# CC834/Heterogeneous-OpenCL-Image-Processing-Engine

Hardware: AMD Instinct MI355X
Metric: images_per_sec (higher is better)
Workload: dtype u8

## Files before the change

heterogeneous-opencl-image-processing-engine_amd/csrc/blur_launch.h:

```cpp
#pragma once
#include <hip/hip_runtime.h>
#include <stdint.h>

#include "filter.h"

namespace mi_blur {

struct LaunchDesc {
    const Filter *filter;
    const uint8_t *in;
    uint8_t *out;
    int width, band_rows, channels;
    int n_images;
    int y0, y1;
    long long in_stride, out_stride;
    int concurrent;
    int max_blocks;
    int variant;
    const uint8_t *halo_top, *halo_bottom;
    hipStream_t stream;
    hipEvent_t start, stop;
};

int launch(const LaunchDesc &d);
// ... 23 lines not shown
constexpr unsigned ZC_PARAM_WORDS = 32;
constexpr unsigned ZC_TRACE_BATCHES = 512;
constexpr unsigned long long ZC_HARD_TICKS = 1000000000ull;
struct ZcBatch {
    unsigned params[ZC_PARAM_WORDS];
    unsigned tile_first;
    unsigned n_tiles;
    unsigned pad[6];
};
struct ZcHostCtl {
    unsigned tail;
    unsigned quit;
    unsigned servers_done;
    unsigned error;
    unsigned pad0[12];
    unsigned done[ZC_RING];
    unsigned long long t_begin[ZC_RING], t_end[ZC_RING];
    ZcBatch batch[ZC_RING];
};
struct ZcDevCtl {
    unsigned next[2];
    unsigned gnext[2];
    unsigned start_seq;
    unsigned avail;
    unsigned stop_seq, stop_at, stop_tile;
    unsigned ticket;
    unsigned pad[6];
    unsigned tiles_done[ZC_RING];
    ZcBatch batch[ZC_RING];
};
struct ZcGeometry { unsigned threads; size_t lds; int rpg; int channels, radius, ragged; };
int zc_fill_batch(const LaunchDesc &d, ZcGeometry *geo, ZcBatch *b, unsigned *n_tiles);
int zc_launch_server(const ZcGeometry &geo, ZcHostCtl *ctl, ZcDevCtl *dev, unsigned seq, unsigned n_workers, unsigned budget,
                     unsigned idle_ticks, hipStream_t stream, unsigned long long *trace = nullptr, int fixed_share = 0);

const char *last_kernel();

bool tiled_eligible(const void *in, const void *out, int width, int channels);

struct Tunables {
    int stage_dma; int rpg; int xcd_remap; int debug_copy; int row_shuffle; int prefer_stream; int stream_bh; int zero_copy; int ragged;
    int fused_release;
    int experiment;
    int xcd_run;
    int zero_copy_streams;
    int zero_copy_blocks;
    int stream_updown;
    int prefer_direct;
    int direct_bh;
    int debug_xcd_times;
    int fused_window;
    int fused_tail;
    int fused_adds_per_word;
    int fused_tail_blocks;
    int zero_copy_server;
    int zero_copy_server_min_kb;
    int staged_server;
    int zero_copy_workers;
    int zero_copy_idle_us;
    int zero_copy_budget;
    int zero_copy_tickets;
    int resident_place_trials;
    int zero_copy_spin;
    int zero_copy_trace;
    int zero_copy_debug_base;
    int zero_copy_events;
};
enum class KnobKind { FLAG, RANGE, ONE_OF };
struct Knob { const char *key; int Tunables::*field; KnobKind kind; int lo, hi, def; const char *env; };
constexpr int knob_bits(int a, int b, int c, int d) { return 1 << a | 1 << b | 1 << c | 1 << d; }
static constexpr Knob KNOBS[] = {
    {"stage_dma", &Tunables::stage_dma, KnobKind::FLAG, 0, 1, 1, "MI_BLUR_STAGE"},
    {"rows_per_thread", &Tunables::rpg, KnobKind::ONE_OF, knob_bits(0, 4, 8, 16), 0, 0, "MI_BLUR_RPG"},
    {"xcd_remap", &Tunables::xcd_remap, KnobKind::FLAG, 0, 1, 1, "MI_BLUR_XCD"},
    {"debug_copy", &Tunables::debug_copy, KnobKind::FLAG, 0, 1, 0, nullptr},
    {"row_shuffle", &Tunables::row_shuffle, KnobKind::FLAG, 0, 1, 0, nullptr},
    {"prefer_stream", &Tunables::prefer_stream, KnobKind::FLAG, 0, 1, 0, nullptr},
    {"zero_copy", &Tunables::zero_copy, KnobKind::FLAG, 0, 1, 1, nullptr},
    {"ragged_tiled", &Tunables::ragged, KnobKind::FLAG, 0, 1, 1, nullptr},
    {"stream_band_rows", &Tunables::stream_bh, KnobKind::RANGE, 0, 4096, 0, nullptr},
    {"fused_release", &Tunables::fused_release, KnobKind::FLAG, 0, 1, 0, nullptr},
    {"experiment", &Tunables::experiment, KnobKind::FLAG, 0, 1, 0, nullptr},
    {"stream_updown", &Tunables::stream_updown, KnobKind::FLAG, 0, 1, 1, nullptr},
    {"zero_copy_streams", &Tunables::zero_copy_streams, KnobKind::RANGE, 1, 8, 4, nullptr},
    {"zero_copy_blocks", &Tunables::zero_copy_blocks, KnobKind::RANGE, 0, 1 << 20, 24, nullptr},
    {"prefer_direct", &Tunables::prefer_direct, KnobKind::RANGE, 0, 2, 1, "MI_BLUR_DIRECT"},
    {"direct_bh", &Tunables::direct_bh, KnobKind::ONE_OF, knob_bits(4, 8, 12, 16), 0, 8, nullptr},
    {"fused_adds_per_word", &Tunables::fused_adds_per_word, KnobKind::RANGE, 4, 4096, 32, nullptr},
    {"fused_tail_blocks", &Tunables::fused_tail_blocks, KnobKind::RANGE, 10, 800, 25, nullptr},
    {"fused_tail", &Tunables::fused_tail, KnobKind::RANGE, 0, 500, 30, "MI_BLUR_FUSED_TAIL"},
    {"fused_window", &Tunables::fused_window, KnobKind::RANGE, 1, 4096, 8, nullptr},
    {"debug_xcd_times", &Tunables::debug_xcd_times, KnobKind::FLAG, 0, 1, 0, nullptr},
    {"zero_copy_events", &Tunables::zero_copy_events, KnobKind::FLAG, 0, 1, 1, nullptr},
    {"zero_copy_server", &Tunables::zero_copy_server, KnobKind::FLAG, 0, 1, 1, nullptr},
    {"staged_server", &Tunables::staged_server, KnobKind::FLAG, 0, 1, 1, "MI_BLUR_STAGED_SERVER"},
    {"zero_copy_server_min_kb", &Tunables::zero_copy_server_min_kb, KnobKind::RANGE, 0, 1 << 20, 1280, nullptr},
    {"zero_copy_trace", &Tunables::zero_copy_trace, KnobKind::FLAG, 0, 1, 0, nullptr},
    {"zero_copy_tickets", &Tunables::zero_copy_tickets, KnobKind::FLAG, 0, 1, 1, nullptr},
    {"zero_copy_spin", &Tunables::zero_copy_spin, KnobKind::FLAG, 0, 1, 0, nullptr},
    {"zero_copy_debug_base", &Tunables::zero_copy_debug_base, KnobKind::RANGE, 0, 1 << 20, 0, nullptr},
    {"resident_place_trials", &Tunables::resident_place_trials, KnobKind::RANGE, 0, 8, 4, "MI_BLUR_PLACE_TRIALS"},
    {"zero_copy_workers", &Tunables::zero_copy_workers, KnobKind::RANGE, 1, 2048, 48, nullptr},
    {"zero_copy_idle_us", &Tunables::zero_copy_idle_us, KnobKind::RANGE, 10, 100000, 300, nullptr},
    {"zero_copy_budget", &Tunables::zero_copy_budget, KnobKind::RANGE, 1, 1 << 20, 256, nullptr},
    {"xcd_run", &Tunables::xcd_run, KnobKind::RANGE, 0, 1 << 20, 0, nullptr},
};
static inline bool knob_set(const Knob &k, Tunables &t, int value)
{
    switch (k.kind) {
    case KnobKind::FLAG: t.*k.field = value != 0; return true;
    case KnobKind::RANGE: if (value < k.lo || value > k.hi) return false; break;
    case KnobKind::ONE_OF: if (value < 0 || value > 30 || !((k.lo >> value) & 1)) return false; break;
    }
    t.*k.field = value;
    return true;
}

Tunables tunables();
unsigned long long *debug_xcd_buffer();
unsigned debug_xcd_slots();
void set_tunables(const Tunables &t);

}
```

heterogeneous-opencl-image-processing-engine_amd/csrc/mi_blur_api.cpp:

```cpp
#include "../../include/mi_blur.h"
#include "blur_launch.h"
#include "cpu_device.h"

#include <hip/hip_runtime.h>
#include <rccl/rccl.h>

#include <dlfcn.h>
#include <sched.h>
#include <time.h>

#include <algorithm>
#include <chrono>
#include <climits>
#include <cmath>
#include <cstdio>
#include <cstdlib>
#include <cstring>
#include <mutex>
#include <new>
#include <deque>
#include <functional>
#include <condition_variable>
#include <thread>
#include <vector>
// ... 296 lines not shown
                j = q.front(); q.pop_front();
            }
            const auto t0 = std::chrono::steady_clock::now();
            j->work();
            const double ms = std::chrono::duration<double, std::milli>(std::chrono::steady_clock::now() - t0).count();
            { std::lock_guard<std::mutex> lk(m); j->ms = ms; j->done = true; }
            cv_done.notify_all();
        }
    }
    void push(CpuJob *j)
    {
        { std::lock_guard<std::mutex> lk(m); q.push_back(j); }
        if (!th.joinable()) th = std::thread([this] { loop(); });
        cv_work.notify_one();
    }
    void wait(CpuJob *j)
    {
        std::unique_lock<std::mutex> lk(m);
        cv_done.wait(lk, [&] { return j->done; });
    }
    ~CpuWorker()
    {
        { std::lock_guard<std::mutex> lk(m); stop = true; }
        cv_work.notify_all();
        if (th.joinable()) th.join();
    }
};

}

struct mi_blur_ctx {
    int device = 0, W = 0, H = 0, C = 0, max_batch = 0, n_threads = 0;
    Filter filter{};
    size_t image_bytes = 0;
    std::vector<Slot> slots;
    int next_slot = 0;
    mi_blur_timing tm{};
    uint8_t *pool_in = nullptr, *pool_out = nullptr;
    int pool_images = 0;
    long long cursor = 0;
    int rr = 0;
    std::vector<TimedLaunch> ev_pool;
    size_t ev_used = 0;
    uint64_t timed_launches = 0, timed_bytes_alg = 0;
    uint64_t zero_copy_launches = 0;
    hipEvent_t zc_ref = nullptr;
    bool zc_ref_valid = false;
    double zc_covered_ms = 0.0;
    unsigned *fused_count = nullptr, *fused_host = nullptr;
    int fused_cap = 0, fused_batches = 0;
    unsigned fused_tpb = 0, fused_wpb = 0, fused_blocks = 0;
    unsigned fused_k = 8;
    int fused_n = 0, fused_batch = 0;
    unsigned fused_passes = 0;
    hipStream_t fused_poll = nullptr;
    hipStream_t fused_watch = nullptr;
    unsigned long long *fused_word = nullptr, *fused_word_dev = nullptr;
    unsigned fused_watch_seq = 0;
    bool fused_watched = false;
    ZcServer *zc = nullptr;
    std::vector<float> place_ms;
    int place_kept = 0;
    std::vector<CpuJob *> cpu_jobs;
    CpuWorker *cpu_worker = nullptr;
    bool submitted = false;
    bool is_cpu() const { return device == MI_BLUR_DEVICE_CPU; }
};

static bool is_pinned(const void *p)
{
    hipPointerAttribute_t a;
    if (hipPointerGetAttributes(&a, p) != hipSuccess) { (void)hipGetLastError(); return false; }
    return a.type == hipMemoryTypeHost;
}

static uint8_t *pinned_device_ptr(const void *p)
{
    hipPointerAttribute_t a;
    if (hipPointerGetAttributes(&a, p) != hipSuccess) { (void)hipGetLastError(); return nullptr; }
    return a.type == hipMemoryTypeHost ? (uint8_t *)a.devicePointer : nullptr;
}

extern "C" void *mi_blur_host_alloc(size_t bytes)
{
    void *p = nullptr;
    if (mi_blur_device_count() > 0) {
        if (hipHostMalloc(&p, bytes, hipHostMallocPortable | hipHostMallocMapped) == hipSuccess) return p;
        (void)hipGetLastError();
        return nullptr;
    }
    return malloc(bytes);
}

extern "C" int mi_blur_host_register(void *p, size_t bytes)
{
    if (!p || bytes == 0) return MI_BLUR_ERR_INVALID;
    if (mi_blur_device_count() <= 0) return MI_BLUR_OK;
    HIP_TRY(hipHostRegister(p, bytes, hipHostRegisterPortable | hipHostRegisterMapped));
    return MI_BLUR_OK;
}

extern "C" int mi_blur_host_unregister(void *p)
{
    if (!p) return MI_BLUR_ERR_INVALID;
    if (mi_blur_device_count() <= 0) return MI_BLUR_OK;
    HIP_TRY(hipHostUnregister(p));
    return MI_BLUR_OK;
// ... 85 lines not shown
    void *p = nullptr;
    if (hipHostMalloc(&p, bytes, hipHostMallocPortable | hipHostMallocMapped) != hipSuccess) { (void)hipGetLastError(); p = nullptr; }
    if (bound > 0 && have_saved) (void)sched_setaffinity(0, sizeof saved, &saved);
    (void)hipSetDevice(prev);
    return p;
}

static void free_slot(Slot &s)
{
    if (s.h_in) (void)hipHostFree(s.h_in);
    if (s.h_out) (void)hipHostFree(s.h_out);
    if (s.d_in) (void)hipFree(s.d_in);
    if (s.d_out) (void)hipFree(s.d_out);
    for (auto &e : s.ev) if (e) (void)hipEventDestroy(e);
    if (s.ks) (void)hipEventDestroy(s.ks);
    if (s.ke) (void)hipEventDestroy(s.ke);
    if (s.stream) (void)hipStreamDestroy(s.stream);
    s = Slot{};
}

extern "C" int mi_blur_create(mi_blur_ctx **out_ctx, int device, int width, int height, int channels, int radius,
                              int max_batch, int n_slots, int n_threads)
{
    if (!out_ctx) return MI_BLUR_ERR_INVALID;
    *out_ctx = nullptr;
    if (width <= 0 || height <= 0 || channels <= 0 || max_batch <= 0 || n_slots <= 0) return MI_BLUR_ERR_INVALID;
    Filter box;
    if (filter_box(radius, &box)) return MI_BLUR_ERR_INVALID;
    if ((long long)width * channels * height > 0x7fffffffLL) return MI_BLUR_ERR_INVALID;
    mi_blur_ctx *c = new (std::nothrow) mi_blur_ctx;
    if (!c) return MI_BLUR_ERR_NOMEM;
    c->device = device; c->W = width; c->H = height; c->C = channels; c->filter = box;
    c->max_batch = max_batch;
    c->n_threads = n_threads > 0 ? n_threads : std::min(hardware_threads(), 16);
    c->image_bytes = (size_t)width * height * channels;
    if (device == MI_BLUR_DEVICE_CPU) { *out_ctx = c; return MI_BLUR_OK; }

    const int ndev = mi_blur_device_count();
    if (ndev <= 0 || device < 0 || device >= ndev) { delete c; return MI_BLUR_ERR_NO_DEVICE; }
    int rc = MI_BLUR_OK;
    auto fail = [&](hipError_t e) { (void)hipGetLastError(); rc = MI_BLUR_ERR_HIP_BASE - (int)e; return true; };
    hipError_t e = hipSetDevice(device);
    if (e != hipSuccess) { fail(e); delete c; return rc; }
    c->slots.resize(n_slots);
    for (auto &s : c->slots) {
        if ((e = hipStreamCreateWithFlags(&s.stream, hipStreamNonBlocking)) != hipSuccess && fail(e)) break;
        for (auto &ev : s.ev) if ((e = hipEventCreate(&ev)) != hipSuccess && fail(e)) break;
        if (rc) break;
        if ((e = hipEventCreate(&s.ks)) != hipSuccess && fail(e)) break;
        if ((e = hipEventCreate(&s.ke)) != hipSuccess && fail(e)) break;
    }
    if (rc) { mi_blur_destroy(c); return rc; }
    *out_ctx = c;
    return MI_BLUR_OK;
}

static int slot_staging(mi_blur_ctx *c, Slot &s, bool in, bool out)
{
    const size_t bytes = c->image_bytes * (size_t)c->max_batch;
    if (in && !s.h_in) HIP_TRY(hipHostMalloc((void **)&s.h_in, bytes, hipHostMallocDefault));
    if (out && !s.h_out) HIP_TRY(hipHostMalloc((void **)&s.h_out, bytes, hipHostMallocDefault));
    return MI_BLUR_OK;
}
static int slot_device(mi_blur_ctx *c, Slot &s)
{
    const size_t bytes = c->image_bytes * (size_t)c->max_batch;
    if (!s.d_in) HIP_TRY(hipMalloc((void **)&s.d_in, bytes));
    if (!s.d_out) HIP_TRY(hipMalloc((void **)&s.d_out, bytes));
    return MI_BLUR_OK;
}

static int finish_slot(mi_blur_ctx *c, Slot &s)
{
    if (!s.busy) return MI_BLUR_OK;
    float ms = 0.f;
    if (s.zero_copy && s.zc_server) {
        ZcServer &z = *c->zc;
        const unsigned slot = s.zc_index % ZC_RING, want = s.zc_index + 1u;
        const auto t0 = std::chrono::steady_clock::now();
        const bool spin_only = tunables().zero_copy_spin != 0;
        for (unsigned spins = 0; __atomic_load_n(&z.ctl->done[slot], __ATOMIC_ACQUIRE) != want; spins++) {
            if (spins < 2048) { __builtin_ia32_pause(); continue; }
            if (__atomic_load_n(&z.ctl->error, __ATOMIC_ACQUIRE)) return MI_BLUR_ERR_STATE;
            if (spin_only) std::this_thread::yield();
            else { struct timespec ts = {0, 20000}; nanosleep(&ts, nullptr); }
            if ((spins & 63u) == 0) {
                const hipError_t q = hipStreamQuery(z.stream);
                if (q != hipSuccess && q != hipErrorNotReady) { (void)hipGetLastError(); return MI_BLUR_ERR_HIP_BASE - (int)q; }
                (void)hipGetLastError();
                if (std::chrono::steady_clock::now() - t0 > std::chrono::seconds(30)) return MI_BLUR_ERR_STATE;
            }
        }
        const unsigned long long b = __atomic_load_n(&z.ctl->t_begin[slot], __ATOMIC_RELAXED), e = __atomic_load_n(&z.ctl->t_end[slot], __ATOMIC_RELAXED);
        if (e >= b) {
            const unsigned long long from = std::max(b, z.covered);
            if (e > from) c->tm.kernel_ms += (double)(e - from) / 1e5;
            z.covered = std::max(z.covered, e);
        }
        if (s.out_staged)
            copy_blocks(s.user_out, s.out_stride, s.h_out, s.out_band, s.out_band, s.out_n, STAGING_COPY_THREADS);
        s.zero_copy = false; s.zc_server = false; s.busy = false;
        return MI_BLUR_OK;
    }
    if (s.zero_copy) {
        if (s.zc_plain) {
            HIP_TRY(hipStreamSynchronize(s.zc_stream));
            s.zero_copy = false; s.busy = false; s.zc_plain = false;
            return MI_BLUR_OK;
        }
        HIP_TRY(hipEventSynchronize(s.ke));
        float a = 0.f, b = 0.f;
        if (c->zc_ref_valid && hipEventElapsedTime(&a, c->zc_ref, s.ks) == hipSuccess && hipEventElapsedTime(&b, c->zc_ref, s.ke) == hipSuccess && b >= a) {
            const double from = std::max((double)a, c->zc_covered_ms);
            if ((double)b > from) c->tm.kernel_ms += (double)b - from;
            c->zc_covered_ms = std::max(c->zc_covered_ms, (double)b);
        } else if (hipEventElapsedTime(&ms, s.ks, s.ke) == hipSuccess) {
            c->tm.kernel_ms += ms;
        }
        (void)hipGetLastError();
        s.zero_copy = false;
        s.busy = false;
        return MI_BLUR_OK;
    }
    HIP_TRY(hipStreamSynchronize(s.stream));
    if (s.out_staged)
        copy_blocks(s.user_out, s.out_stride, s.h_out, s.out_band, s.out_band, s.out_n, STAGING_COPY_THREADS);
    if (hipEventElapsedTime(&ms, s.ev[0], s.ev[1]) == hipSuccess) c->tm.h2d_ms += ms;
    if (hipEventElapsedTime(&ms, s.ks, s.ke) == hipSuccess) c->tm.kernel_ms += ms;
    if (hipEventElapsedTime(&ms, s.ev[2], s.ev[3]) == hipSuccess) c->tm.d2h_ms += ms;
    (void)hipGetLastError();
    s.busy = false;
    return MI_BLUR_OK;
}

static int harvest_resident(mi_blur_ctx *c)
{
    for (size_t i = 0; i < c->ev_used; i++) {
        float ms = 0.f;
        if (hipEventElapsedTime(&ms, c->ev_pool[i].s, c->ev_pool[i].e) == hipSuccess) c->tm.kernel_ms += ms;
    }
    (void)hipGetLastError();
    c->ev_used = 0;
    return MI_BLUR_OK;
}

extern "C" int mi_blur_sync(mi_blur_ctx *c, mi_blur_timing *timing)
{
    if (!c) return MI_BLUR_ERR_INVALID;
    if (c->is_cpu()) {
        for (CpuJob *j : c->cpu_jobs) {
            c->cpu_worker->wait(j);
            c->tm.kernel_ms += j->ms;
            delete j;
        }
        c->cpu_jobs.clear();
    } else {
        HIP_TRY(hipSetDevice(c->device));
        for (auto &s : c->slots) {
            int rc = finish_slot(c, s);
            if (rc) return rc;
        }
        for (auto &s : c->slots) HIP_TRY(hipStreamSynchronize(s.stream));
        if (c->fused_watched && c->fused_watch) HIP_TRY(hipStreamSynchronize(c->fused_watch));
        harvest_resident(c);
        c->zc_ref_valid = false;
    }
    if (timing) *timing = c->tm;
    return MI_BLUR_OK;
}

extern "C" int mi_blur_get_timing(mi_blur_ctx *c, mi_blur_timing *timing)
{
    if (!c || !timing) return MI_BLUR_ERR_INVALID;
    *timing = c->tm;
    return MI_BLUR_OK;
}

extern "C" uint64_t mi_blur_zero_copy_launches(mi_blur_ctx *c) { return c ? c->zero_copy_launches : 0; }

extern "C" void mi_blur_reset_timing(mi_blur_ctx *c)
{
    if (!c) return;
    c->tm = mi_blur_timing{};
    c->timed_launches = 0; c->timed_bytes_alg = 0;
}

extern "C" void mi_blur_timed_coverage(mi_blur_ctx *c, uint64_t *launches, uint64_t *bytes_alg)
{
    if (launches) *launches = c ? c->timed_launches : 0;
    if (bytes_alg) *bytes_alg = c ? c->timed_bytes_alg : 0;
}

extern "C" void mi_blur_destroy(mi_blur_ctx *c)
{
    if (!c) return;
    for (CpuJob *j : c->cpu_jobs) { c->cpu_worker->wait(j); delete j; }
    delete c->cpu_worker;
    if (!c->is_cpu()) {
        (void)hipSetDevice(c->device);
        for (auto &s : c->slots) { if (s.stream) (void)hipStreamSynchronize(s.stream); }
        if (c->zc) {
            ZcServer &z = *c->zc;
            if (z.ctl) __atomic_store_n(&z.ctl->quit, 1u, __ATOMIC_RELEASE);
            if (getenv("MI_BLUR_DEBUG_SERVER"))
                fprintf(stderr, "[mi_blur] destroy: server state head %u launched %u servers_done %u tail %u; stream query %d\n", z.head, z.launched,
                        z.ctl ? z.ctl->servers_done : 0u, z.ctl ? z.ctl->tail : 0u, z.stream ? (int)hipStreamQuery(z.stream) : -1);
            if (z.stream) { (void)hipStreamSynchronize(z.stream); (void)hipStreamDestroy(z.stream); }
            if (getenv("MI_BLUR_DEBUG_SERVER")) fprintf(stderr, "[mi_blur] destroy: servers gone\n");
            if (z.dev) (void)hipFree(z.dev);
            if (z.trace) (void)hipFree(z.trace);
            if (z.ctl) (void)hipHostFree(z.ctl);
            delete c->zc;
            c->zc = nullptr;
        }
        for (auto &s : c->slots) free_slot(s);
        for (auto &t : c->ev_pool) { (void)hipEventDestroy(t.s); (void)hipEventDestroy(t.e); }
        if (c->zc_ref) (void)hipEventDestroy(c->zc_ref);
        if (c->fused_count) (void)hipFree(c->fused_count);
        if (c->fused_host) (void)hipHostFree(c->fused_host);
        if (c->fused_poll) { (void)hipStreamSynchronize(c->fused_poll); (void)hipStreamDestroy(c->fused_poll); }
        if (c->fused_watch) { (void)hipStreamSynchronize(c->fused_watch); (void)hipStreamDestroy(c->fused_watch); }
        if (c->fused_word) (void)hipHostFree(c->fused_word);
        if (c->pool_in) (void)hipFree(c->pool_in);
        if (c->pool_out) (void)hipFree(c->pool_out);
        (void)hipGetLastError();
    }
    delete c;
}

static int zc_server_submit(mi_blur_ctx *c, Slot &s, const LaunchDesc &d, const Tunables &tun)
{
    if (c->filter.kind != FilterKind::BOX) return MI_BLUR_ERR_UNSUPPORTED;
    if (c->slots.size() > ZC_RING) return MI_BLUR_ERR_UNSUPPORTED;
    if (!c->zc) {
        ZcServer *z = new (std::nothrow) ZcServer;
        if (!z) return MI_BLUR_ERR_NOMEM;
        hipError_t e = hipHostMalloc((void **)&z->ctl, sizeof(ZcHostCtl), hipHostMallocDefault);
        if (e == hipSuccess) { memset(z->ctl, 0, sizeof(ZcHostCtl)); e = hipHostGetDevicePointer((void **)&z->ctl_dev, z->ctl, 0); }
        if (e == hipSuccess) e = hipStreamCreateWithFlags(&z->stream, hipStreamNonBlocking);
        if (e == hipSuccess) e = hipMalloc((void **)&z->dev, sizeof(ZcDevCtl));
        if (e == hipSuccess) e = hipMemsetAsync(z->dev, 0, sizeof(ZcDevCtl), z->stream);
        if (e == hipSuccess && tun.zero_copy_trace) {
            const size_t tb = (size_t)ZC_TRACE_BATCHES * (size_t)tun.zero_copy_workers * 5u * sizeof(unsigned long long);
            e = hipMalloc((void **)&z->trace, tb);
            if (e == hipSuccess) e = hipMemsetAsync(z->trace, 0, tb, z->stream);
        }
        if (e == hipSuccess && tun.zero_copy_debug_base > 0) {
            const unsigned B = 0u - (unsigned)tun.zero_copy_debug_base, T = 0u - 7u * (unsigned)tun.zero_copy_debug_base;
            ZcDevCtl init{};
            init.next[0] = B; init.gnext[0] = T; init.avail = B; init.ticket = T;
            e = hipMemcpyAsync(z->dev, &init, offsetof(ZcDevCtl, tiles_done), hipMemcpyHostToDevice, z->stream);
            if (e == hipSuccess) e = hipStreamSynchronize(z->stream);
            z->ctl->tail = B;
// ... 126 lines not shown
    uint8_t *zout = pinned_device_ptr(s.out_staged ? s.h_out : b.out);
    if (!zin || !zout) return MI_BLUR_ERR_UNSUPPORTED;
    LaunchDesc d = ctx_launch(c, zin, zout, b.band_rows, b.n_images, b.y0, b.y1);
    d.in_stride = (long long)src_stride; d.out_stride = (long long)(s.out_staged ? b.band_out : b.out_stride);
    return submit_to_server(c, s, b, d, tun);
}

static int submit_dma(mi_blur_ctx *c, Slot &s, const HostBatch &b, const uint8_t *src, size_t src_stride)
{
    int rc = slot_device(c, s);
    if (rc) return rc;
    HIP_TRY(hipEventRecord(s.ev[0], s.stream));
    if (src_stride == b.band_in)
        HIP_TRY(hipMemcpyAsync(s.d_in, src, b.in_bytes(), hipMemcpyHostToDevice, s.stream));
    else
        HIP_TRY(hipMemcpy2DAsync(s.d_in, b.band_in, src, src_stride, b.band_in, (size_t)b.n_images, hipMemcpyHostToDevice, s.stream));
    HIP_TRY(hipEventRecord(s.ev[1], s.stream));
    LaunchDesc d = ctx_launch(c, s.d_in, s.d_out, b.band_rows, b.n_images, b.y0, b.y1);
    d.stream = s.stream; d.start = s.ks; d.stop = s.ke;
    d.concurrent = (int)c->slots.size();
    rc = launch(d);
    if (rc) return rc;
    HIP_TRY(hipEventRecord(s.ev[2], s.stream));
    if (s.out_staged || b.out_stride == b.band_out)
        HIP_TRY(hipMemcpyAsync(s.out_staged ? s.h_out : b.out, s.d_out, b.out_bytes(), hipMemcpyDeviceToHost, s.stream));
    else
        HIP_TRY(hipMemcpy2DAsync(b.out, b.out_stride, s.d_out, b.band_out, b.band_out, (size_t)b.n_images, hipMemcpyDeviceToHost, s.stream));
    HIP_TRY(hipEventRecord(s.ev[3], s.stream));
    s.busy = true;
    count_submit(c, b.n_images, b.out_bytes(), b.in_bytes(), b.out_bytes(), false);
    return MI_BLUR_OK;
}

static int submit_common(mi_blur_ctx *c, const uint8_t *host_in, uint8_t *host_out, int band_rows, int n_images,
                         int y0, int y1, size_t in_stride, size_t out_stride)
{
    const size_t pitch = (size_t)c->W * c->C;
    const size_t band_in = pitch * band_rows, band_out = pitch * (size_t)(y1 - y0);
    const HostBatch b{host_in, host_out, band_rows, n_images, y0, y1, band_in, band_out,
                      in_stride ? in_stride : band_in, out_stride ? out_stride : band_out};
    c->submitted = true;
    if (c->is_cpu()) {
        const int W = c->W, C = c->C, nt = c->n_threads;
        const int rc = cpu_enqueue(c, [=, f = c->filter]() {
            cpu_blur_batch(b.in, b.out, W, band_rows, C, f, n_images, y0, y1, nt, b.in_stride, b.out_stride);
        });
        if (rc) return rc;
        count_submit(c, n_images, b.out_bytes(), 0, 0, false);
        return MI_BLUR_OK;
    }
    HIP_TRY(hipSetDevice(c->device));
    Slot &s = c->slots[c->next_slot];
    c->next_slot = (c->next_slot + 1) % (int)c->slots.size();
    int rc = finish_slot(c, s);
    if (rc) return rc;
    const Tunables tun = tunables();
    if (tun.zero_copy) {
        const uint8_t *zin = pinned_device_ptr(host_in);
        uint8_t *zout = pinned_device_ptr(host_out);
        const bool dense = b.in_stride == band_in && b.out_stride == band_out;
        if (zin && zout && (dense || (tiled_eligible(zin, zout, c->W, c->C) && b.in_stride % 16 == 0 && b.out_stride % 16 == 0)))
            return submit_in_place(c, s, b, zin, zout, tun);
    }
    const bool in_pinned = is_pinned(host_in);
    s.zero_copy = false;
    s.out_staged = !is_pinned(host_out);
    s.user_out = host_out; s.out_bytes = b.out_bytes(); s.out_band = band_out; s.out_stride = b.out_stride; s.out_n = n_images;
    const uint8_t *src = host_in;
    size_t src_stride = b.in_stride;
    rc = slot_staging(c, s, !in_pinned, s.out_staged);
    if (rc) return rc;
    if (!in_pinned) {
        copy_blocks(s.h_in, band_in, host_in, b.in_stride, band_in, n_images, STAGING_COPY_THREADS);
        src = s.h_in; src_stride = band_in;
    }
    if (tun.zero_copy && tun.zero_copy_server && tun.staged_server) {
        rc = submit_staged_server(c, s, b, src, src_stride, tun);
        if (rc != MI_BLUR_ERR_UNSUPPORTED) return rc;
    }
    return submit_dma(c, s, b, src, src_stride);
}

extern "C" int mi_blur_submit(mi_blur_ctx *c, const uint8_t *host_in, uint8_t *host_out, int n_images)
{
    if (!c || !host_in || !host_out || host_in == host_out) return MI_BLUR_ERR_INVALID;
    if (n_images < 0 || n_images > c->max_batch) return MI_BLUR_ERR_INVALID;
    if (n_images == 0) return MI_BLUR_OK;
    return submit_common(c, host_in, host_out, c->H, n_images, 0, c->H, 0, 0);
}

extern "C" int mi_blur_submit_band(mi_blur_ctx *c, const uint8_t *host_in, uint8_t *host_out, int band_rows,
                                   int halo_top, int halo_bottom)
{
    if (!c || !host_in || !host_out || host_in == host_out) return MI_BLUR_ERR_INVALID;
    if (band_rows <= 0 || band_rows > c->H || halo_top < 0 || halo_bottom < 0) return MI_BLUR_ERR_INVALID;
    if (halo_top + halo_bottom >= band_rows) return MI_BLUR_ERR_INVALID;
    return submit_common(c, host_in, host_out, band_rows, 1, halo_top, band_rows - halo_bottom, 0, 0);
}

extern "C" int mi_blur_submit_bands(mi_blur_ctx *c, const uint8_t *host_in, uint8_t *host_out, int n_images,
                                    size_t host_image_stride, int band_rows, int halo_top, int halo_bottom)
{
    if (!c || !host_in || !host_out || host_in == host_out) return MI_BLUR_ERR_INVALID;
    if (n_images < 0 || n_images > c->max_batch) return MI_BLUR_ERR_INVALID;
    if (band_rows <= 0 || band_rows > c->H || halo_top < 0 || halo_bottom < 0) return MI_BLUR_ERR_INVALID;
    if (halo_top + halo_bottom >= band_rows) return MI_BLUR_ERR_INVALID;
    if (host_image_stride < (size_t)c->W * c->C * band_rows) return MI_BLUR_ERR_INVALID;
// ... 145 lines not shown
    c->place_ms.clear();
    int keep_in = 0, keep_out = 0;
    if (n_ok > 1) {
        hipStream_t st = c->slots[0].stream;
        hipEvent_t e0 = nullptr, e1 = nullptr;
        std::vector<float> best((size_t)n_ok * n_ok, 1e30f);
        if (hipEventCreate(&e0) == hipSuccess && hipEventCreate(&e1) == hipSuccess) {
            auto pass = [&](int i, int j) {
                LaunchDesc d = ctx_launch(c, in[i], out[j], c->H, pool_images, 0, c->H);
                d.stream = st;
                return launch(d);
            };
            int rc = MI_BLUR_OK;
            const auto t0 = std::chrono::steady_clock::now();
            while (rc == MI_BLUR_OK && std::chrono::steady_clock::now() - t0 < std::chrono::milliseconds(50)) {
                for (int r = 0; r < 4 && rc == MI_BLUR_OK; r++) rc = pass(0, 0);
                if (hipStreamSynchronize(st) != hipSuccess) rc = MI_BLUR_ERR_STATE;
            }
            for (int round = 0; round < 2 && rc == MI_BLUR_OK; round++)
                for (int i = 0; i < n_ok && rc == MI_BLUR_OK; i++)
                    for (int j = 0; j < n_ok && rc == MI_BLUR_OK; j++) {
                        rc = pass(i, j);
                        (void)hipEventRecord(e0, st);
                        for (int r = 0; r < 2 && rc == MI_BLUR_OK; r++) rc = pass(i, j);
                        (void)hipEventRecord(e1, st);
                        float ms = 0.f;
                        if (hipEventSynchronize(e1) == hipSuccess && hipEventElapsedTime(&ms, e0, e1) == hipSuccess && ms > 0.f)
                            best[(size_t)i * n_ok + j] = std::min(best[(size_t)i * n_ok + j], ms / 2.0f);
                    }
            (void)hipGetLastError();
            for (int i = 0; i < n_ok; i++)
                for (int j = 0; j < n_ok; j++) {
                    c->place_ms.push_back(best[(size_t)i * n_ok + j]);
                    if (best[(size_t)i * n_ok + j] < best[(size_t)keep_in * n_ok + keep_out]) { keep_in = i; keep_out = j; }
                }
        }
        if (e0) (void)hipEventDestroy(e0);
        if (e1) (void)hipEventDestroy(e1);
    }
    c->pool_in = in[keep_in]; c->pool_out = out[keep_out];
    c->place_kept = keep_in * n_ok + keep_out;
    for (int i = 0; i < trials; i++) {
        if (i != keep_in && in[i]) (void)hipFree(in[i]);
        if (i != keep_out && out[i]) (void)hipFree(out[i]);
    }
    return MI_BLUR_OK;
}

extern "C" int mi_blur_resident_alloc(mi_blur_ctx *c, int pool_images)
{
    if (!c || pool_images <= 0) return MI_BLUR_ERR_INVALID;
    if (c->is_cpu()) return MI_BLUR_ERR_STATE;
    HIP_TRY(hipSetDevice(c->device));
    if (c->pool_in) { (void)hipFree(c->pool_in); c->pool_in = nullptr; }
    if (c->pool_out) { (void)hipFree(c->pool_out); c->pool_out = nullptr; }
    c->pool_images = 0; c->cursor = 0;
    const size_t bytes = c->image_bytes * (size_t)pool_images;
    const int trials = tunables().resident_place_trials;
    if (trials > 1 && bytes >= ((size_t)128 << 20) && bytes <= ((size_t)8 << 30)) {
        int rc = place_pool(c, bytes, pool_images, std::min(trials, 8));
        if (rc) return rc;
    } else {
        c->place_ms.clear(); c->place_kept = 0;
        HIP_TRY(hipMalloc((void **)&c->pool_in, bytes));
        HIP_TRY(hipMalloc((void **)&c->pool_out, bytes));
    }
    c->pool_images = pool_images;
    return MI_BLUR_OK;
}

extern "C" int mi_blur_resident_placement(mi_blur_ctx *c, float *ms, int max_n, int *kept)
{
    if (!c) return MI_BLUR_ERR_INVALID;
    const int n = (int)std::min<size_t>(c->place_ms.size(), (size_t)std::max(max_n, 0));
    for (int i = 0; i < n && ms; i++) ms[i] = c->place_ms[i];
    if (kept) *kept = c->place_kept;
    return n;
}

extern "C" int mi_blur_resident_upload(mi_blur_ctx *c, int pool_index, const uint8_t *host_in, int n_images)
{
    if (!c || !host_in || !c->pool_in) return MI_BLUR_ERR_STATE;
    if (pool_index < 0 || n_images < 0 || pool_index + n_images > c->pool_images) return MI_BLUR_ERR_INVALID;
    HIP_TRY(hipSetDevice(c->device));
    HIP_TRY(hipMemcpy(c->pool_in + (size_t)pool_index * c->image_bytes, host_in, c->image_bytes * (size_t)n_images,
                      hipMemcpyHostToDevice));
    return MI_BLUR_OK;
}

extern "C" int mi_blur_resident_download(mi_blur_ctx *c, int pool_index, uint8_t *host_out, int n_images)
{
    if (!c || !host_out || !c->pool_out) return MI_BLUR_ERR_STATE;
    if (pool_index < 0 || n_images < 0 || pool_index + n_images > c->pool_images) return MI_BLUR_ERR_INVALID;
    HIP_TRY(hipSetDevice(c->device));
    HIP_TRY(hipDeviceSynchronize());
    HIP_TRY(hipMemcpy(host_out, c->pool_out + (size_t)pool_index * c->image_bytes, c->image_bytes * (size_t)n_images,
                      hipMemcpyDeviceToHost));
    return MI_BLUR_OK;
}

extern "C" int mi_blur_resident_fill_synthetic(mi_blur_ctx *c, int first_index)
{
    if (!c || !c->pool_in) return MI_BLUR_ERR_STATE;
    const int chunk = std::max(1, (int)std::min<size_t>((size_t)c->pool_images, ((size_t)256 << 20) / c->image_bytes));
    std::vector<uint8_t> host;
    try { host.resize(c->image_bytes * (size_t)chunk); } catch (...) { return MI_BLUR_ERR_NOMEM; }
    for (int i = 0; i < c->pool_images; i += chunk) {
        const int n = std::min(chunk, c->pool_images - i);
        fill_synthetic(host.data(), c->W, c->H, c->C, first_index + i, n, c->n_threads);
        int rc = mi_blur_resident_upload(c, i, host.data(), n);
        if (rc) return rc;
    }
    return MI_BLUR_OK;
}

extern "C" void *mi_blur_resident_in(mi_blur_ctx *c) { return c ? c->pool_in : nullptr; }
extern "C" void *mi_blur_resident_out(mi_blur_ctx *c) { return c ? c->pool_out : nullptr; }

extern "C" int mi_blur_resident_run(mi_blur_ctx *c, int n_images, int batch, int timed_every)
{
    if (!c || n_images < 0 || batch <= 0) return MI_BLUR_ERR_INVALID;
    if (c->filter.kind != FilterKind::BOX) return MI_BLUR_ERR_UNSUPPORTED;
    if (c->is_cpu() || !c->pool_in) return MI_BLUR_ERR_STATE;
    if (batch > c->pool_images) return MI_BLUR_ERR_INVALID;
    HIP_TRY(hipSetDevice(c->device));
    int launch_idx = 0;
    for (int done = 0; done < n_images; done += batch, launch_idx++) {
        const int b = std::min(batch, n_images - done);
        const bool timed = timed_every > 0 && launch_idx % timed_every == 0;
        if (c->cursor + b > c->pool_images) c->cursor = 0;
        Slot &s = c->slots[c->rr];
        c->rr = (c->rr + 1) % (int)c->slots.size();
        LaunchDesc d = ctx_launch(c, c->pool_in + (size_t)c->cursor * c->image_bytes, c->pool_out + (size_t)c->cursor * c->image_bytes,
                                  c->H, b, 0, c->H);
        d.stream = s.stream;
        d.concurrent = (int)c->slots.size();
        if (timed) {
            if (c->ev_used == c->ev_pool.size()) {
                TimedLaunch t{};
                HIP_TRY(hipEventCreate(&t.s));
                HIP_TRY(hipEventCreate(&t.e));
                c->ev_pool.push_back(t);
            }
            d.start = c->ev_pool[c->ev_used].s; d.stop = c->ev_pool[c->ev_used].e;
            c->ev_used++;
        }
        int rc = launch(d);
        if (rc) return rc;
        c->cursor += b;
        c->tm.launches += 1;
        if (timed) { c->timed_launches += 1; c->timed_bytes_alg += 2ull * c->image_bytes * (uint64_t)b; }
    }
    c->tm.images += (uint64_t)n_images;
    c->tm.bytes_alg += 2ull * c->image_bytes * (uint64_t)n_images;
    return MI_BLUR_OK;
}

static size_t fused_words(int cap) { return 8 * (size_t)cap + 16384; }

extern "C" int mi_blur_resident_run_fused(mi_blur_ctx *c, int n_images, int batch, int timed)
{
    if (!c || n_images <= 0 || batch <= 0) return MI_BLUR_ERR_INVALID;
    if (c->filter.kind != FilterKind::BOX) return MI_BLUR_ERR_UNSUPPORTED;
    if (c->is_cpu() || !c->pool_in) return MI_BLUR_ERR_STATE;
    if (n_images > c->pool_images) return MI_BLUR_ERR_INVALID;
    HIP_TRY(hipSetDevice(c->device));
    const int nb = (n_images + batch - 1) / batch;
    if (nb > c->fused_cap) {
        for (auto &s : c->slots) HIP_TRY(hipStreamSynchronize(s.stream));
        if (c->fused_count) { (void)hipFree(c->fused_count); c->fused_count = nullptr; }
        if (c->fused_host) { (void)hipHostFree(c->fused_host); c->fused_host = nullptr; }
        c->fused_cap = 0;
        const int cap = std::max(nb, c->pool_images);
        HIP_TRY(hipMalloc((void **)&c->fused_count, sizeof(unsigned) * (fused_words(cap) + 16)));
        HIP_TRY(hipMemset(c->fused_count + fused_words(cap), 0, sizeof(unsigned) * 16));
        HIP_TRY(hipDeviceSynchronize());
        HIP_TRY(hipHostMalloc((void **)&c->fused_host, sizeof(unsigned) * fused_words(cap), hipHostMallocDefault));
        c->fused_cap = cap;
        c->fused_passes = 0;
    }
    if (!c->fused_poll) {
        HIP_TRY(hipStreamCreateWithFlags(&c->fused_poll, hipStreamNonBlocking));
        HIP_TRY(hipMemcpyAsync(c->fused_host, c->fused_count, sizeof(unsigned) * fused_words(c->fused_cap), hipMemcpyDeviceToHost, c->fused_poll));
        HIP_TRY(hipStreamSynchronize(c->fused_poll));
    }
    if (c->cursor + n_images > c->pool_images) c->cursor = 0;
    Slot &s = c->slots[0];
    LaunchDesc d = ctx_launch(c, c->pool_in + (size_t)c->cursor * c->image_bytes, c->pool_out + (size_t)c->cursor * c->image_bytes,
                              c->H, n_images, 0, c->H);
    d.variant = MI_BLUR_VARIANT_TILED; d.stream = s.stream;
    const Tunables tun = tunables();
    unsigned tpb = 0, wpb = 0, blocks = 0, kcnt = 8;
    FusedDesc f{c->fused_count, batch, &tpb, &wpb, &blocks, &tun, true, c->fused_count + fused_words(c->fused_cap), (long long)fused_words(c->fused_cap), &kcnt};
    int rc = launch_fused(d, f);
    if (rc) return rc;
    if (n_images == c->fused_n && batch == c->fused_batch && tpb == c->fused_tpb && wpb == c->fused_wpb && kcnt == c->fused_k &&
        blocks == c->fused_blocks && c->fused_passes > 0 && c->fused_passes < (1u << 20)) {
        c->fused_passes += 1;
    } else {
        if (c->fused_watched && c->fused_watch) HIP_TRY(hipStreamSynchronize(c->fused_watch));
        HIP_TRY(hipMemsetAsync(c->fused_count, 0, sizeof(unsigned) * (size_t)kcnt * (size_t)nb, s.stream));
        c->fused_n = n_images; c->fused_batch = batch; c->fused_passes = 1;
        c->fused_tpb = tpb; c->fused_wpb = wpb; c->fused_blocks = blocks; c->fused_k = kcnt;
    }
    c->fused_batches = nb;
    c->fused_watched = false;
    if (timed & 2) {
        if (c->fused_passes == 1) HIP_TRY(hipStreamSynchronize(s.stream));
        if (!c->fused_watch) HIP_TRY(hipStreamCreateWithFlags(&c->fused_watch, hipStreamNonBlocking));
        if (!c->fused_word) {
            HIP_TRY(hipHostMalloc((void **)&c->fused_word, sizeof(unsigned long long), hipHostMallocDefault));
            *c->fused_word = 0;
            HIP_TRY(hipHostGetDevicePointer((void **)&c->fused_word_dev, c->fused_word, 0));
        }
        c->fused_watch_seq += 1;
        rc = launch_fused_watch(c->fused_count, (unsigned)nb, tpb, blocks, wpb * c->fused_passes, c->fused_word_dev, c->fused_watch_seq, c->fused_watch, c->fused_k);
        if (rc) return rc;
        c->fused_watched = true;
    }
    if (timed & 1) {
        if (c->ev_used == c->ev_pool.size()) {
            TimedLaunch t{};
            HIP_TRY(hipEventCreate(&t.s));
            HIP_TRY(hipEventCreate(&t.e));
            c->ev_pool.push_back(t);
        }
        d.start = c->ev_pool[c->ev_used].s; d.stop = c->ev_pool[c->ev_used].e;
        c->ev_used++;
    }
    f.geometry_only = false;
    rc = launch_fused(d, f);
    if (rc) { c->fused_passes = 0; c->fused_batches = 0; return rc; }
    c->cursor += n_images;
    c->tm.launches += 1;
    c->tm.images += (uint64_t)n_images;
    c->tm.bytes_alg += 2ull * c->image_bytes * (uint64_t)n_images;
    if (timed & 1) { c->timed_launches += 1; c->timed_bytes_alg += 2ull * c->image_bytes * (uint64_t)n_images; }
    return MI_BLUR_OK;
}

extern "C" int mi_blur_resident_batches_done(mi_blur_ctx *c)
{
    if (!c) return MI_BLUR_ERR_INVALID;
    if (c->is_cpu()) return MI_BLUR_ERR_STATE;
    if (!c->fused_count || !c->fused_batches) return 0;
    if (c->fused_watched) {
        const unsigned long long w = __atomic_load_n(c->fused_word, __ATOMIC_ACQUIRE);
        return (unsigned)(w >> 32) == c->fused_watch_seq ? (int)(unsigned)(w & 0xffffffffu) : 0;
    }
    HIP_TRY(hipSetDevice(c->device));
    const unsigned K = c->fused_k;
    HIP_TRY(hipMemcpyAsync(c->fused_host, c->fused_count, sizeof(unsigned) * (size_t)K * (size_t)c->fused_batches, hipMemcpyDeviceToHost, c->fused_poll));
    HIP_TRY(hipStreamSynchronize(c->fused_poll));
    int n = 0;
    for (; n < c->fused_batches; n++) {
        const unsigned first = (unsigned)n * c->fused_tpb;
        const unsigned blocks = std::min(c->fused_tpb, c->fused_blocks - first);
        unsigned sum = 0;
        for (unsigned k = 0; k < K; k++) sum += c->fused_host[(size_t)K * n + k];
        if (sum != blocks * c->fused_wpb * c->fused_passes) break;
    }
    return n;
}

extern "C" int mi_blur_resident_peek(mi_blur_ctx *c, int pool_index, uint8_t *host_out, int n_images)
{
    if (!c || !host_out || !c->pool_out || !c->fused_poll) return MI_BLUR_ERR_STATE;
    if (pool_index < 0 || n_images < 0 || pool_index + n_images > c->pool_images) return MI_BLUR_ERR_INVALID;
    HIP_TRY(hipSetDevice(c->device));
    HIP_TRY(hipMemcpyAsync(host_out, c->pool_out + (size_t)pool_index * c->image_bytes, c->image_bytes * (size_t)n_images,
                           hipMemcpyDeviceToHost, c->fused_poll));
    HIP_TRY(hipStreamSynchronize(c->fused_poll));
    return MI_BLUR_OK;
}

static int cpu_run_filter(const Filter &f, const uint8_t *in, uint8_t *out, int width, int height, int channels, int n_images,
                          int n_threads)
{
    if (!in || !out || in == out || width <= 0 || height <= 0 || channels <= 0 || n_images < 0)
        return MI_BLUR_ERR_INVALID;
    if (f.kind != FilterKind::BOX && (long long)width * channels * height > INT_MAX) return MI_BLUR_ERR_INVALID;
    cpu_blur_batch(in, out, width, height, channels, f, n_images, 0, height, n_threads);
    return MI_BLUR_OK;
}

extern "C" int mi_blur_cpu_run(const uint8_t *in, uint8_t *out, int width, int height, int channels, int radius,
                               int n_images, int n_threads)
{
    Filter f;
    return filter_box(radius, &f) ? MI_BLUR_ERR_INVALID : cpu_run_filter(f, in, out, width, height, channels, n_images, n_threads);
}

extern "C" int mi_blur_cpu_run_sep(const uint8_t *in, uint8_t *out, int width, int height, int channels, int n_images,
                                   const mi_blur_sep_kernel *k, int n_threads)
{
    Filter f;
    return filter_sep(k, &f) ? MI_BLUR_ERR_INVALID : cpu_run_filter(f, in, out, width, height, channels, n_images, n_threads);
}

extern "C" int mi_blur_cpu_run_median(const uint8_t *in, uint8_t *out, int width, int height, int channels, int radius,
                                      int n_images, int n_threads)
{
    Filter f;
    return filter_median(radius, &f) ? MI_BLUR_ERR_INVALID : cpu_run_filter(f, in, out, width, height, channels, n_images, n_threads);
}

extern "C" int mi_blur_cpu_run_morph(const uint8_t *in, uint8_t *out, int width, int height, int channels, int op, int rx, int ry,
                                     int n_images, int n_threads)
{
    Filter f;
    return filter_morph(op, rx, ry, &f) ? MI_BLUR_ERR_INVALID : cpu_run_filter(f, in, out, width, height, channels, n_images, n_threads);
}

// ... 430 lines not shown
```

Before: 15.00 million.

## Add optional dual-lane fused resident launches and cache fused geometry

Adds a fused_lanes knob (default 1) that alternates fused resident launches between two streams, each with its own completion-counter region, so consecutive passes can overlap. Caches the geometry-only launch_fused result keyed on shape, input pointer and tunables, skipping the repeated geometry query. Pre-reserves timing events in bulk instead of creating them on demand. Adds join/synchronization points across the API to keep the second lane coherent, at the cost of extra sync calls and more state.

```diff
diff --git a/heterogeneous-opencl-image-processing-engine_amd/csrc/blur_launch.h b/heterogeneous-opencl-image-processing-engine_amd/csrc/blur_launch.h
--- a/heterogeneous-opencl-image-processing-engine_amd/csrc/blur_launch.h
+++ b/heterogeneous-opencl-image-processing-engine_amd/csrc/blur_launch.h
@@ -99,6 +99,7 @@
     int fused_window;
     int fused_tail;
     int fused_adds_per_word;
+    int fused_lanes;
     int fused_tail_blocks;
     int zero_copy_server;
     int zero_copy_server_min_kb;
@@ -137,6 +138,7 @@
     {"fused_tail_blocks", &Tunables::fused_tail_blocks, KnobKind::RANGE, 10, 800, 25, nullptr},
     {"fused_tail", &Tunables::fused_tail, KnobKind::RANGE, 0, 500, 30, "MI_BLUR_FUSED_TAIL"},
     {"fused_window", &Tunables::fused_window, KnobKind::RANGE, 1, 4096, 8, nullptr},
+    {"fused_lanes", &Tunables::fused_lanes, KnobKind::RANGE, 1, 2, 1, "MI_BLUR_FUSED_LANES"},
     {"debug_xcd_times", &Tunables::debug_xcd_times, KnobKind::FLAG, 0, 1, 0, nullptr},
     {"zero_copy_events", &Tunables::zero_copy_events, KnobKind::FLAG, 0, 1, 1, nullptr},
     {"zero_copy_server", &Tunables::zero_copy_server, KnobKind::FLAG, 0, 1, 1, nullptr},
diff --git a/heterogeneous-opencl-image-processing-engine_amd/csrc/mi_blur_api.cpp b/heterogeneous-opencl-image-processing-engine_amd/csrc/mi_blur_api.cpp
--- a/heterogeneous-opencl-image-processing-engine_amd/csrc/mi_blur_api.cpp
+++ b/heterogeneous-opencl-image-processing-engine_amd/csrc/mi_blur_api.cpp
@@ -372,7 +372,12 @@
     unsigned fused_tpb = 0, fused_wpb = 0, fused_blocks = 0;
     unsigned fused_k = 8;
     int fused_n = 0, fused_batch = 0;
-    unsigned fused_passes = 0;
+    hipStream_t fused_lane1 = nullptr;
+    bool fused_lane1_owned = false;
+    unsigned fused_passes[2] = {0, 0};
+    bool fused_lane1_pending = false;
+    int fused_lane = 1;
+    struct FusedGeo { bool valid = false; int n = 0, batch = 0, radius = 0; const uint8_t *in = nullptr; Tunables tun{}; unsigned tpb = 0, wpb = 0, blocks = 0, k = 8; } fused_geo;
     hipStream_t fused_poll = nullptr;
     hipStream_t fused_watch = nullptr;
     unsigned long long *fused_word = nullptr, *fused_word_dev = nullptr;
@@ -564,6 +569,25 @@
     }
     if (rc) { mi_blur_destroy(c); return rc; }
     *out_ctx = c;
+    return MI_BLUR_OK;
+}
+
+static int fused_join(mi_blur_ctx *c)
+{
+    if (!c->fused_lane1_pending) return MI_BLUR_OK;
+    HIP_TRY(hipStreamSynchronize(c->fused_lane1));
+    c->fused_lane1_pending = false;
+    return MI_BLUR_OK;
+}
+
+static int ev_reserve(mi_blur_ctx *c, size_t n)
+{
+    while (c->ev_pool.size() < n) {
+        TimedLaunch t{};
+        HIP_TRY(hipEventCreate(&t.s));
+        if (hipEventCreate(&t.e) != hipSuccess) { (void)hipEventDestroy(t.s); (void)hipGetLastError(); return MI_BLUR_ERR_STATE; }
+        c->ev_pool.push_back(t);
+    }
     return MI_BLUR_OK;
 }
 
@@ -652,6 +676,7 @@
         if (hipEventElapsedTime(&ms, c->ev_pool[i].s, c->ev_pool[i].e) == hipSuccess) c->tm.kernel_ms += ms;
     }
     (void)hipGetLastError();
+    if (c->ev_used && c->ev_used == c->ev_pool.size() && c->ev_pool.size() < 65536) (void)ev_reserve(c, 2 * c->ev_pool.size());
     c->ev_used = 0;
     return MI_BLUR_OK;
 }
@@ -673,6 +698,7 @@
             if (rc) return rc;
         }
         for (auto &s : c->slots) HIP_TRY(hipStreamSynchronize(s.stream));
+        { int rc = fused_join(c); if (rc) return rc; }
         if (c->fused_watched && c->fused_watch) HIP_TRY(hipStreamSynchronize(c->fused_watch));
         harvest_resident(c);
         c->zc_ref_valid = false;
@@ -693,6 +719,10 @@
 extern "C" void mi_blur_reset_timing(mi_blur_ctx *c)
 {
     if (!c) return;
+    if (!c->is_cpu() && c->fused_lane1_pending && hipSetDevice(c->device) == hipSuccess) {
+        (void)hipStreamSynchronize(c->slots[0].stream);
+        (void)fused_join(c);
+    }
     c->tm = mi_blur_timing{};
     c->timed_launches = 0; c->timed_bytes_alg = 0;
 }
@@ -711,6 +741,7 @@
     if (!c->is_cpu()) {
         (void)hipSetDevice(c->device);
         for (auto &s : c->slots) { if (s.stream) (void)hipStreamSynchronize(s.stream); }
+        if (c->fused_lane1) { (void)hipStreamSynchronize(c->fused_lane1); if (c->fused_lane1_owned) (void)hipStreamDestroy(c->fused_lane1); c->fused_lane1 = nullptr; }
         if (c->zc) {
             ZcServer &z = *c->zc;
             if (z.ctl) __atomic_store_n(&z.ctl->quit, 1u, __ATOMIC_RELEASE);
@@ -943,7 +974,9 @@
     HIP_TRY(hipSetDevice(c->device));
     Slot &s = c->slots[c->next_slot];
     c->next_slot = (c->next_slot + 1) % (int)c->slots.size();
-    int rc = finish_slot(c, s);
+    int rc = fused_join(c);
+    if (rc) return rc;
+    rc = finish_slot(c, s);
     if (rc) return rc;
     const Tunables tun = tunables();
     if (tun.zero_copy) {
@@ -1195,6 +1228,12 @@
     if (!c || pool_images <= 0) return MI_BLUR_ERR_INVALID;
     if (c->is_cpu()) return MI_BLUR_ERR_STATE;
     HIP_TRY(hipSetDevice(c->device));
+    if (c->fused_lane1_pending) {
+        HIP_TRY(hipStreamSynchronize(c->slots[0].stream));
+        int rc = fused_join(c);
+        if (rc) return rc;
+    }
+    c->fused_geo.valid = false;
     if (c->pool_in) { (void)hipFree(c->pool_in); c->pool_in = nullptr; }
     if (c->pool_out) { (void)hipFree(c->pool_out); c->pool_out = nullptr; }
     c->pool_images = 0; c->cursor = 0;
@@ -1209,7 +1248,7 @@
         HIP_TRY(hipMalloc((void **)&c->pool_out, bytes));
     }
     c->pool_images = pool_images;
-    return MI_BLUR_OK;
+    return ev_reserve(c, 256);
 }
 
 extern "C" int mi_blur_resident_placement(mi_blur_ctx *c, float *ms, int max_n, int *kept)
@@ -1226,6 +1265,11 @@
     if (!c || !host_in || !c->pool_in) return MI_BLUR_ERR_STATE;
     if (pool_index < 0 || n_images < 0 || pool_index + n_images > c->pool_images) return MI_BLUR_ERR_INVALID;
     HIP_TRY(hipSetDevice(c->device));
+    if (c->fused_lane1_pending) {
+        HIP_TRY(hipStreamSynchronize(c->slots[0].stream));
+        int rc = fused_join(c);
+        if (rc) return rc;
+    }
     HIP_TRY(hipMemcpy(c->pool_in + (size_t)pool_index * c->image_bytes, host_in, c->image_bytes * (size_t)n_images,
                       hipMemcpyHostToDevice));
     return MI_BLUR_OK;
@@ -1237,6 +1281,7 @@
     if (pool_index < 0 || n_images < 0 || pool_index + n_images > c->pool_images) return MI_BLUR_ERR_INVALID;
     HIP_TRY(hipSetDevice(c->device));
     HIP_TRY(hipDeviceSynchronize());
+    c->fused_lane1_pending = false;
     HIP_TRY(hipMemcpy(host_out, c->pool_out + (size_t)pool_index * c->image_bytes, c->image_bytes * (size_t)n_images,
                       hipMemcpyDeviceToHost));
     return MI_BLUR_OK;
@@ -1267,6 +1312,7 @@
     if (c->is_cpu() || !c->pool_in) return MI_BLUR_ERR_STATE;
     if (batch > c->pool_images) return MI_BLUR_ERR_INVALID;
     HIP_TRY(hipSetDevice(c->device));
+    { int rc = fused_join(c); if (rc) return rc; }
     int launch_idx = 0;
     for (int done = 0; done < n_images; done += batch, launch_idx++) {
         const int b = std::min(batch, n_images - done);
@@ -1279,12 +1325,7 @@
         d.stream = s.stream;
         d.concurrent = (int)c->slots.size();
         if (timed) {
-            if (c->ev_used == c->ev_pool.size()) {
-                TimedLaunch t{};
-                HIP_TRY(hipEventCreate(&t.s));
-                HIP_TRY(hipEventCreate(&t.e));
-                c->ev_pool.push_back(t);
-            }
+            if (c->ev_used == c->ev_pool.size()) { int rc = ev_reserve(c, c->ev_used + 1); if (rc) return rc; }
             d.start = c->ev_pool[c->ev_used].s; d.stop = c->ev_pool[c->ev_used].e;
             c->ev_used++;
         }
@@ -1300,6 +1341,8 @@
 }
 
 static size_t fused_words(int cap) { return 8 * (size_t)cap + 16384; }
+static size_t fused_lane_words(int cap) { return fused_words(cap) + 16; }
+static unsigned *fused_lane_count(const mi_blur_ctx *c, int lane) { return c->fused_count + (size_t)lane * fused_lane_words(c->fused_cap); }
 
 extern "C" int mi_blur_resident_run_fused(mi_blur_ctx *c, int n_images, int batch, int timed)
 {
@@ -1311,16 +1354,20 @@
     const int nb = (n_images + batch - 1) / batch;
     if (nb > c->fused_cap) {
         for (auto &s : c->slots) HIP_TRY(hipStreamSynchronize(s.stream));
+        { int rc = fused_join(c); if (rc) return rc; }
+        if (c->fused_watched && c->fused_watch) HIP_TRY(hipStreamSynchronize(c->fused_watch));
         if (c->fused_count) { (void)hipFree(c->fused_count); c->fused_count = nullptr; }
         if (c->fused_host) { (void)hipHostFree(c->fused_host); c->fused_host = nullptr; }
         c->fused_cap = 0;
         const int cap = std::max(nb, c->pool_images);
-        HIP_TRY(hipMalloc((void **)&c->fused_count, sizeof(unsigned) * (fused_words(cap) + 16)));
+        HIP_TRY(hipMalloc((void **)&c->fused_count, sizeof(unsigned) * 2 * fused_lane_words(cap)));
         HIP_TRY(hipMemset(c->fused_count + fused_words(cap), 0, sizeof(unsigned) * 16));
+        HIP_TRY(hipMemset(c->fused_count + fused_lane_words(cap) + fused_words(cap), 0, sizeof(unsigned) * 16));
         HIP_TRY(hipDeviceSynchronize());
         HIP_TRY(hipHostMalloc((void **)&c->fused_host, sizeof(unsigned) * fused_words(cap), hipHostMallocDefault));
         c->fused_cap = cap;
-        c->fused_passes = 0;
+        c->fused_passes[0] = c->fused_passes[1] = 0;
+        c->fused_batches = 0; c->fused_watched = false;
     }
     if (!c->fused_poll) {
         HIP_TRY(hipStreamCreateWithFlags(&c->fused_poll, hipStreamNonBlocking));
@@ -1328,28 +1375,59 @@
         HIP_TRY(hipStreamSynchronize(c->fused_poll));
     }
     if (c->cursor + n_images > c->pool_images) c->cursor = 0;
-    Slot &s = c->slots[0];
-    LaunchDesc d = ctx_launch(c, c->pool_in + (size_t)c->cursor * c->image_bytes, c->pool_out + (size_t)c->cursor * c->image_bytes,
-                              c->H, n_images, 0, c->H);
-    d.variant = MI_BLUR_VARIANT_TILED; d.stream = s.stream;
+    const uint8_t *in = c->pool_in + (size_t)c->cursor * c->image_bytes;
+    LaunchDesc d = ctx_launch(c, in, c->pool_out + (size_t)c->cursor * c->image_bytes, c->H, n_images, 0, c->H);
+    d.variant = MI_BLUR_VARIANT_TILED;
     const Tunables tun = tunables();
     unsigned tpb = 0, wpb = 0, blocks = 0, kcnt = 8;
-    FusedDesc f{c->fused_count, batch, &tpb, &wpb, &blocks, &tun, true, c->fused_count + fused_words(c->fused_cap), (long long)fused_words(c->fused_cap), &kcnt};
-    int rc = launch_fused(d, f);
-    if (rc) return rc;
-    if (n_images == c->fused_n && batch == c->fused_batch && tpb == c->fused_tpb && wpb == c->fused_wpb && kcnt == c->fused_k &&
-        blocks == c->fused_blocks && c->fused_passes > 0 && c->fused_passes < (1u << 20)) {
-        c->fused_passes += 1;
+    FusedDesc f{nullptr, batch, &tpb, &wpb, &blocks, &tun, true, nullptr, (long long)fused_words(c->fused_cap), &kcnt};
+    auto &g = c->fused_geo;
+    int rc = MI_BLUR_OK;
+    if (g.valid && g.n == n_images && g.batch == batch && g.radius == c->filter.radius && g.in == in && !memcmp(&g.tun, &tun, sizeof tun)) {
+        tpb = g.tpb; wpb = g.wpb; blocks = g.blocks; kcnt = g.k;
+    } else {
+        f.count = c->fused_count; f.tail_ctr = c->fused_count + fused_words(c->fused_cap);
+        rc = launch_fused(d, f);
+        if (rc) return rc;
+        g.valid = true; g.n = n_images; g.batch = batch; g.radius = c->filter.radius; g.in = in; g.tun = tun;
+        g.tpb = tpb; g.wpb = wpb; g.blocks = blocks; g.k = kcnt;
+    }
+    if (!(n_images == c->fused_n && batch == c->fused_batch && tpb == c->fused_tpb && wpb == c->fused_wpb && kcnt == c->fused_k &&
+          blocks == c->fused_blocks)) {
+        if (c->fused_lane1_pending) {
+            HIP_TRY(hipStreamSynchronize(c->slots[0].stream));
+            rc = fused_join(c);
+            if (rc) return rc;
+        }
+        if (c->fused_watched && c->fused_watch) HIP_TRY(hipStreamSynchronize(c->fused_watch));
+        c->fused_passes[0] = c->fused_passes[1] = 0;
+        c->fused_n = n_images; c->fused_batch = batch;
+        c->fused_tpb = tpb; c->fused_wpb = wpb; c->fused_blocks = blocks; c->fused_k = kcnt;
+    }
+    const int lane = tun.fused_lanes >= 2 ? (c->fused_lane ^ 1) : 0;
+    if (lane == 0 && tun.fused_lanes < 2) { rc = fused_join(c); if (rc) return rc; }
+    if (lane && !c->fused_lane1) {
+        if (c->slots.size() >= 2) c->fused_lane1 = c->slots[1].stream;
+        else { HIP_TRY(hipStreamCreateWithFlags(&c->fused_lane1, hipStreamNonBlocking)); c->fused_lane1_owned = true; }
+    }
+    const hipStream_t stream = lane ? c->fused_lane1 : c->slots[0].stream;
+    unsigned *count = fused_lane_count(c, lane);
+    d.stream = stream;
+    f.count = count; f.tail_ctr = count + fused_words(c->fused_cap);
+    unsigned &passes = c->fused_passes[lane];
+    if (passes > 0 && passes < (1u << 20)) {
+        passes += 1;
     } else {
         if (c->fused_watched && c->fused_watch) HIP_TRY(hipStreamSynchronize(c->fused_watch));
-        HIP_TRY(hipMemsetAsync(c->fused_count, 0, sizeof(unsigned) * (size_t)kcnt * (size_t)nb, s.stream));
-        c->fused_n = n_images; c->fused_batch = batch; c->fused_passes = 1;
-        c->fused_tpb = tpb; c->fused_wpb = wpb; c->fused_blocks = blocks; c->fused_k = kcnt;
+        HIP_TRY(hipMemsetAsync(count, 0, sizeof(unsigned) * (size_t)kcnt * (size_t)nb, stream));
+        passes = 1;
     }
     c->fused_batches = nb;
+    c->fused_lane = lane;
     c->fused_watched = false;
-    if (timed & 2) {
-        if (c->fused_passes == 1) HIP_TRY(hipStreamSynchronize(s.stream));
+    if (lane) c->fused_lane1_pending = true;
+    auto watch = [&]() -> int {
+        if (passes == 1) HIP_TRY(hipStreamSynchronize(stream));
         if (!c->fused_watch) HIP_TRY(hipStreamCreateWithFlags(&c->fused_watch, hipStreamNonBlocking));
         if (!c->fused_word) {
             HIP_TRY(hipHostMalloc((void **)&c->fused_word, sizeof(unsigned long long), hipHostMallocDefault));
@@ -1357,23 +1435,22 @@
             HIP_TRY(hipHostGetDevicePointer((void **)&c->fused_word_dev, c->fused_word, 0));
         }
         c->fused_watch_seq += 1;
-        rc = launch_fused_watch(c->fused_count, (unsigned)nb, tpb, blocks, wpb * c->fused_passes, c->fused_word_dev, c->fused_watch_seq, c->fused_watch, c->fused_k);
-        if (rc) return rc;
+        const int wrc = launch_fused_watch(count, (unsigned)nb, tpb, blocks, wpb * passes, c->fused_word_dev, c->fused_watch_seq, c->fused_watch, c->fused_k);
+        if (wrc) return wrc;
         c->fused_watched = true;
-    }
+        return MI_BLUR_OK;
+    };
+    const bool watch_first = tun.fused_lanes < 2;
+    if ((timed & 2) && watch_first) { rc = watch(); if (rc) return rc; }
     if (timed & 1) {
-        if (c->ev_used == c->ev_pool.size()) {
-            TimedLaunch t{};
-            HIP_TRY(hipEventCreate(&t.s));
-            HIP_TRY(hipEventCreate(&t.e));
-            c->ev_pool.push_back(t);
-        }
+        if (c->ev_used == c->ev_pool.size()) { rc = ev_reserve(c, c->ev_used + 1); if (rc) return rc; }
         d.start = c->ev_pool[c->ev_used].s; d.stop = c->ev_pool[c->ev_used].e;
         c->ev_used++;
     }
     f.geometry_only = false;
     rc = launch_fused(d, f);
-    if (rc) { c->fused_passes = 0; c->fused_batches = 0; return rc; }
+    if (rc) { passes = 0; c->fused_batches = 0; return rc; }
+    if ((timed & 2) && !watch_first) { rc = watch(); if (rc) return rc; }
     c->cursor += n_images;
     c->tm.launches += 1;
     c->tm.images += (uint64_t)n_images;
@@ -1393,7 +1470,7 @@
     }
     HIP_TRY(hipSetDevice(c->device));
     const unsigned K = c->fused_k;
-    HIP_TRY(hipMemcpyAsync(c->fused_host, c->fused_count, sizeof(unsigned) * (size_t)K * (size_t)c->fused_batches, hipMemcpyDeviceToHost, c->fused_poll));
+    HIP_TRY(hipMemcpyAsync(c->fused_host, fused_lane_count(c, c->fused_lane), sizeof(unsigned) * (size_t)K * (size_t)c->fused_batches, hipMemcpyDeviceToHost, c->fused_poll));
     HIP_TRY(hipStreamSynchronize(c->fused_poll));
     int n = 0;
     for (; n < c->fused_batches; n++) {
@@ -1401,7 +1478,7 @@
         const unsigned blocks = std::min(c->fused_tpb, c->fused_blocks - first);
         unsigned sum = 0;
         for (unsigned k = 0; k < K; k++) sum += c->fused_host[(size_t)K * n + k];
-        if (sum != blocks * c->fused_wpb * c->fused_passes) break;
+        if (sum != blocks * c->fused_wpb * c->fused_passes[c->fused_lane]) break;
     }
     return n;
 }
```

Result: slower. 14.81 million (-1.3%).
